# mcogoni/supersdr

Measured on AMD Instinct MI355X. Metric: real-time IQ channels sustained (WF+demod), higher is better.
Workload: dtype f32

## Files before the change

supersdr_amd/csrc/ssdr_wf.hip:

```cpp
#include "ssdr_math.h"
#include "ssdr_kernels.h"
#include "ssdr_audio_dev.h"
#include "ssdr_wf_dev.h"

namespace {

constexpr int WAVES = SSDR_WF_BLOCK / 64;
constexpr int LDS_TOTAL = LDS_XCH + WAVES * 2 * XCH_FLOATS * 4;
static_assert(LDS_TOTAL <= 163840, "LDS budget");
constexpr int LDS_SCAN = LDS_TOTAL;
constexpr int LDS_SCAN_BYTES = 6 * 64 * 4;
constexpr int LDS_TOTAL_FUSED = LDS_SCAN + LDS_SCAN_BYTES;
static_assert(LDS_SCAN % 4 == 0 && 2 * LDS_TOTAL_FUSED <= 163840, "two workgroups per CU");

template <bool AVG, bool HOP>
__global__ __launch_bounds__(SSDR_WF_BLOCK, SSDR_WF_WAVES_PER_EU) void ssdr_wf_kernel(SsdrWfArgs a)
{
    __shared__ __attribute__((aligned(16))) unsigned char smem[LDS_TOTAL];
    load_tables(smem, a.win, a.tw_stage, a.lut);

    const int lane = threadIdx.x & 63, wave = __builtin_amdgcn_readfirstlane(threadIdx.x >> 6);
    const int h = lane >> 5, l = lane & 31;
    float *xch_wave = reinterpret_cast<float *>(smem + LDS_XCH) + wave * 2 * XCH_FLOATS;
    const unsigned char *lut = smem + LDS_LUT0;
    const uint32_t n_pairs = (a.n_ch + 1) >> 1;
    const uint32_t run = HOP ? a.grp_run : 1u;
    const uint32_t n_runs = (a.n_groups + run - 1) / run;
    const uint32_t n_items = n_pairs * n_runs;
    const uint32_t wave_stride = gridDim.x * WAVES;

    for (uint32_t item = blockIdx.x * WAVES + wave; item < n_items; item += wave_stride) {
      uint32_t pair, g_begin, g_end;
      if (HOP) {
          pair = item / n_runs;
          g_begin = (item - pair * n_runs) * run;
          g_end = min(g_begin + run, a.n_groups);
      } else {
          g_begin = item / n_pairs;
          pair = item - g_begin * n_pairs;
          g_end = g_begin + 1;
      }
      const uint32_t n_trips = HOP ? g_end - g_begin : 1u;
      for (uint32_t trip = 0; trip < n_trips; trip++) {
        const uint32_t grp = g_begin + trip;
        uint32_t pair_now = __builtin_amdgcn_readfirstlane(pair);
        asm volatile("" : "+s"(pair_now));
        const WfItem it = wf_item(a, pair_now, grp, h);
        const float calq = a.consts[it.ch].wf_cal_lin * SSDR_LUT_SCALE;
        uint32_t acc[AVG ? 16 : 1];
#pragma unroll
        for (int j = 0; j < (AVG ? 16 : 1); j++) acc[j] = 0;
        constexpr uint32_t LINE_STEP = HOP ? SSDR_NFFT / 2 : SSDR_NFFT;
        const uint32_t *src = a.iq + (uint64_t)it.ch * a.ch_stride + (uint64_t)it.l0 * LINE_STEP + l;

        for (uint32_t line = it.l0; line < it.l1; line++, src += LINE_STEP) {
            f32x2 z[32];
            uint32_t raw[32];
            if (HOP) load_line_halves(line ? src - SSDR_NFFT / 2 : a.tail + (uint64_t)it.ch * (SSDR_NFFT / 2) + l, src, raw);
            else load_line(src, raw);
            if (SSDR_PRIO_WF) prio_compute_phase();
            window_line(raw, smem, l, z);
            SCHED_FENCE();
            fft_line<AVG>(z, smem, xch_wave, h, l);
            if (SSDR_PRIO_WF) prio_latency_phase();

            if (AVG) {
                quantise32(z, calq, lut, [&](int j, uint32_t q01) { acc[j] += q01; });
            } else {
                uint32_t q[16];
                quantise32(z, calq, lut, [&](int j, uint32_t q01) { q[j] = q01; });
                int16_t *x16 = reinterpret_cast<int16_t *>(xch_wave + opaque(h) * XCH_FLOATS) + opaque(l);
#pragma unroll
                for (int j = 0; j < 16; j++) {
                    x16[32 * (j + 16)] = (int16_t)(q[j] & 0xFFFFu);
                    x16[32 * j] = (int16_t)(q[j] >> 16);
                }
            }
        }

        float *xch = xch_wave + opaque(h) * XCH_FLOATS;
        if (AVG) {
            int16_t *x16 = reinterpret_cast<int16_t *>(xch) + opaque(l);
#pragma unroll
            for (int j = 0; j < 16; j++) {
                x16[32 * (j + 16)] = (int16_t)(acc[j] & 0xFFFFu);
                x16[32 * j] = (int16_t)(acc[j] >> 16);
            }
        }
        wave_lds_sync();
        const u32x4 *x128 = reinterpret_cast<const u32x4 *>(xch);
        int16_t *dst = it.complete ? a.out + ((uint64_t)it.grp * a.n_ch + it.ch) * SSDR_NFFT
                                   : a.acc_out + (uint64_t)it.ch * SSDR_NFFT;
        const int16_t *cin = a.acc_in + (uint64_t)it.ch * SSDR_NFFT;
#pragma unroll
        for (int q = 0; q < 4; q++) {
            u32x4 v = x128[q * 32 + l];
// ... 2 lines not shown
            if (it.ch_ok) SSDR_NT_STORE(v, reinterpret_cast<u32x4 *>(dst) + q * 32 + l);
        }
        wave_lds_sync();
      }
    }
}

template <typename T>
SSDR_DEV u32x4 *lane_at(T *base, uint32_t lane_bytes)
{
    return reinterpret_cast<u32x4 *>(reinterpret_cast<char *>(base) + lane_bytes);
}
template <typename T>
SSDR_DEV const u32x4 *lane_at(const T *base, uint32_t lane_bytes)
{
    return reinterpret_cast<const u32x4 *>(reinterpret_cast<const char *>(base) + lane_bytes);
}

template <bool HOP, bool AVG = false, bool HANG = true>
__global__ __launch_bounds__(SSDR_WF_BLOCK, SSDR_WF_WAVES_PER_EU) void ssdr_fused_am_kernel(SsdrFusedArgs fa)
{
    __shared__ __attribute__((aligned(16))) unsigned char smem[LDS_TOTAL_FUSED];
    const SsdrWfArgs &a = fa.wf;
    const SsdrAudioArgs &u = fa.au;
    if (threadIdx.x < 64) {
        DcScan t;
        scan_affine_consts(t);
        float *s_scan = reinterpret_cast<float *>(smem + LDS_SCAN) + threadIdx.x;
#pragma unroll
        for (int k = 1; k < 6; k++) s_scan[64 * (k - 1)] = t.a[k];
        s_scan[64 * 5] = t.ae;
    }
    load_tables(smem, a.win, a.tw_stage, a.lut);

    const int lane = threadIdx.x & 63, wave = __builtin_amdgcn_readfirstlane(threadIdx.x >> 6);
    const int h = lane >> 5, l = lane & 31;
    float *xch_wave = reinterpret_cast<float *>(smem + LDS_XCH) + wave * 2 * XCH_FLOATS;
    uint32_t *qbuf = reinterpret_cast<uint32_t *>(xch_wave);
    const unsigned char *lut = smem + LDS_LUT0;
    const uint32_t n_pairs = (a.n_ch + 1) >> 1;
    const uint32_t wave_stride = gridDim.x * WAVES;
    const uint32_t n_frames = u.n_frames;

    for (uint32_t pair = blockIdx.x * WAVES + wave; pair < n_pairs; pair += wave_stride) {
        const uint32_t ch_raw = 2 * pair + h;
        const bool ch_ok = ch_raw < a.n_ch;
        const uint32_t ch = ch_ok ? ch_raw : a.n_ch - 1;
        const float cal_wf = a.consts[ch].wf_cal_lin * SSDR_LUT_SCALE;
        const uint32_t n_sub = (2 * pair + 1 < a.n_ch) ? 2u : 1u;

        float rssi_sum[2] = {0.0f, 0.0f};
        uint32_t flag_keep[2] = {0u, 0u};
        auto pad = [&](int c, int i) -> float & { return xch_wave[c * XCH_FLOATS + 33 * (i + 17) + 32]; };
        constexpr int PAD_TAIL = HANG ? 10 : 2;
        constexpr bool PARKED = !HOP;
        constexpr int PARK = PARKED ? 4 : 0;
        if (lane < 2) {
            const uint32_t cc = min(2 * pair + (uint32_t)lane, a.n_ch - 1);
            const ssdr_chan_state st = u.state[cc];
            pad(lane, 0) = st.dc;
            pad(lane, 1) = st.agc_d;
            if (HANG) {
#pragma unroll
                for (int i = 0; i < 8; i++) pad(lane, 2 + i) = st.agc_m[i];
            }
            const uint4 t = *reinterpret_cast<const uint4 *>(u.hist + (size_t)cc * SSDR_HIST + SSDR_HIST - 4);
            if constexpr (PARKED) {
                pad(lane, PAD_TAIL) = __uint_as_float(t.x); pad(lane, PAD_TAIL + 1) = __uint_as_float(t.y);
                pad(lane, PAD_TAIL + 2) = __uint_as_float(t.z); pad(lane, PAD_TAIL + 3) = __uint_as_float(t.w);
            } else {
                pad(lane, PAD_TAIL) = __uint_as_float(iq_power(t.x)); pad(lane, PAD_TAIL + 1) = __uint_as_float(iq_power(t.y));
                pad(lane, PAD_TAIL + 2) = __uint_as_float(iq_power(t.z)); pad(lane, PAD_TAIL + 3) = __uint_as_float(iq_power(t.w));
            }
        }
        wave_lds_sync();

        const uint32_t *src = a.iq + (uint64_t)ch * a.ch_stride + l;
        uint32_t last_raw31 = 0;
        uint32_t acc[AVG ? 16 : 1];
#pragma unroll
        for (int j = 0; j < (AVG ? 16 : 1); j++) acc[j] = 0;
        constexpr uint32_t LINE_STEP = HOP ? SSDR_NFFT / 2 : SSDR_NFFT;
        constexpr int FRAMES_PER_LINE = HOP ? 1 : 2;
        for (uint32_t line = 0; line < a.n_lines; line++, src += LINE_STEP) {
            float dc[2], agc_d[2];
            AgcHang<HANG> hang[2];
            uint32_t tail_q[2][4];
#pragma unroll
            for (int c = 0; c < 2; c++) {
                dc[c] = pad(c, 0); agc_d[c] = pad(c, 1);
                if constexpr (HANG) {
#pragma unroll
                    for (int i = 0; i < 8; i++) hang[c].m[i] = pad(c, 2 + i);
                }
                if constexpr (!PARKED) {
#pragma unroll
                    for (int i = 0; i < 4; i++) tail_q[c][i] = __float_as_uint(pad(c, PAD_TAIL + i));
                }
            }
            if constexpr (PARKED) {
                u32x4 b[2];
#pragma unroll
                for (int c = 0; c < 2; c++)
#pragma unroll
                    for (int i = 0; i < 4; i++) b[c][i] = __float_as_uint(pad(c, PAD_TAIL + i));
                wave_lds_sync();
                if (lane == 0) {
#pragma unroll
                    for (int c = 0; c < 2; c++) *reinterpret_cast<u32x4 *>(qbuf + c * XCH_FLOATS) = b[c];
                }
            }
            wave_lds_sync();
            const uint32_t lw = opaque(lane);
            uint32_t *q_park = qbuf + PARK + 4 * lw;
            const uint32_t *q_lane = q_park - PARK + 4 * lw, *q_last = qbuf + (lw & 3u);
            const uint32_t lane16 = lw << 4;
            {
                u32x4 t[2][4];
#pragma unroll
                for (int c = 0; c < 2; c++) {
                    uint32_t pair_now = __builtin_amdgcn_readfirstlane(pair);
                    asm volatile("" : "+s"(pair_now));
                    const uint32_t cc = min(2 * pair_now + (uint32_t)c, a.n_ch - 1);
                    const uint32_t *row = a.iq + (uint64_t)cc * a.ch_stride + (uint64_t)line * LINE_STEP;
                    if (HOP) {
                        const uint32_t *older = line ? row - SSDR_NFFT / 2 : a.tail + (uint64_t)cc * (SSDR_NFFT / 2);
#pragma unroll
                        for (int i = 0; i < 2; i++) t[c][i] = SSDR_NT_LOAD(lane_at(older, lane16) + 64 * i);
#pragma unroll
                        for (int i = 0; i < 2; i++) t[c][2 + i] = lane_at(row, lane16)[64 * i];
                    } else {
#pragma unroll
                        for (int i = 0; i < 4; i++) t[c][i] = SSDR_NT_LOAD(lane_at(row, lane16) + 64 * i);
                    }
                }
                SCHED_FENCE();
#pragma unroll
                for (int c = 0; c < 2; c++)
#pragma unroll
                    for (int i = 0; i < 4; i++) reinterpret_cast<u32x4 *>(q_park + c * XCH_FLOATS)[64 * i] = t[c][i];
                SCHED_FENCE();
            }
            wave_lds_sync();
            DcScan dcs;
            {
                constexpr float DC_APOW[8] = SSDR_DC_APOW_INIT;
                uint32_t scan_base = LDS_SCAN;
                asm volatile("" : "+s"(scan_base));
                const float *s_scan = reinterpret_cast<const float *>(smem + scan_base) + lw;
                dcs.a[0] = DC_APOW[7];
                asm volatile("" : "+v"(dcs.a[0]));
#pragma unroll
                for (int k = 1; k < 6; k++) dcs.a[k] = s_scan[64 * (k - 1)];
                dcs.ae = s_scan[64 * 5];
            }
            prio_latency_phase();
#pragma unroll
            for (int c = 0; c < 2; c++) {
                if ((uint32_t)c >= n_sub) continue;
                uint32_t pair_now = __builtin_amdgcn_readfirstlane(pair);
                asm volatile("" : "+s"(pair_now));
                const uint32_t cc = 2 * pair_now + c;
                const ssdr_chan_consts &kc = u.consts[cc];
                const AgcK agc_c = {kc.agc_c0, kc.agc_c1, kc.agc_knee, kc.agc_delta8, kc.hang_frames};
                const float cal_c = kc.smeter_cal_db;
#pragma unroll
                for (int f = 0; f < FRAMES_PER_LINE; f++) {
                    const uint32_t frame = HOP ? line : 2 * line + f;
                    const int FBASE = c * XCH_FLOATS + SSDR_FRAME * (HOP ? 1 : f);
                    const u32x4 *qp = reinterpret_cast<const u32x4 *>(q_lane + FBASE);
                    const u32x4 q0 = qp[0], q1 = qp[1];
                    const uint32_t rw[8] = {q0.x, q0.y, q0.z, q0.w, q1.x, q1.y, q1.z, q1.w};
                    uint32_t d[8];
                    float p[8], aud[8];
                    float pmx;
                    bool trig;
                    uint32_t clip;
                    if constexpr (PARKED) {
                        const uint32_t last = q_last[FBASE + SSDR_FRAME];
#pragma unroll
                        for (int j = 0; j < 8; j++) d[j] = iq_power(rw[j]);
#pragma unroll
                        for (int j = 0; j < 8; j++) p[j] = (float)d[j];
                        pmx = block_peak(p);
                        trig = wave_any((pmx >= 1073676160.0f) | (iq_power(last) >= 0x3FFF0001u));
                        clip = trig ? (wave_count(raw_clipped_delayed(rw, last, lane)) + 63u) >> 6 : 0u;
                    } else {
                        uint32_t qv[8];
#pragma unroll
                        for (int j = 0; j < 8; j++) qv[j] = iq_power(rw[j]);
#pragma unroll
                        for (int j = 0; j < 4; j++) { d[j] = from_prev_lane_u(tail_q[c][j], qv[4 + j]); d[4 + j] = qv[j]; }
#pragma unroll
                        for (int j = 0; j < 4; j++) tail_q[c][j] = lane63_u(qv[4 + j]);
#pragma unroll
                        for (int j = 0; j < 8; j++) p[j] = (float)d[j];
                        pmx = block_peak(p);
                        trig = wave_any(pmx >= 1073676160.0f) || tail_q[c][0] >= 0x3FFF0001u || tail_q[c][1] >= 0x3FFF0001u ||
                               tail_q[c][2] >= 0x3FFF0001u || tail_q[c][3] >= 0x3FFF0001u;
                        clip = trig ? (wave_count(raw_clipped(rw)) + 63u) >> 6 : 0u;
                    }
                    demod_am_tab(p, dc[c], aud, dcs);
                    agc_pack_store_fused<HANG>(aud, lane, agc_c, agc_d[c], hang[c], u.pcm + ((uint64_t)cc * n_frames + frame) * SSDR_FRAME, lane16, pmx);
                    rssi_flag_step_uniform(p, clip, frame, n_frames, lane, cal_c, rssi_sum[c], flag_keep[c],
                                           u.rssi + (uint64_t)cc * n_frames, u.flags + (uint64_t)cc * n_frames);
                }
            }
            wave_lds_sync();
            prio_compute_phase();
            uint32_t raw[32];
            {
                const uint32_t *q = qbuf + opaque(h) * XCH_FLOATS + opaque(l);
#pragma unroll
                for (int r = 0; r < 32; r++) raw[r] = q[PARK + 32 * r];
            }
            wave_lds_sync();
            if (lane < 2) {
#pragma unroll
                for (int c = 0; c < 2; c++) {
                    if (lane != c) continue;
                    pad(c, 0) = dc[c]; pad(c, 1) = agc_d[c];
                    if constexpr (HANG) {
#pragma unroll
                        for (int i = 0; i < 8; i++) pad(c, 2 + i) = hang[c].m[i];
                    }
                    if constexpr (PARKED) {
                        const u32x4 e = *reinterpret_cast<const u32x4 *>(qbuf + c * XCH_FLOATS + PARK + SSDR_NFFT - 4);
#pragma unroll
                        for (int i = 0; i < 4; i++) pad(c, PAD_TAIL + i) = __uint_as_float(e[i]);
                    } else {
#pragma unroll
                        for (int i = 0; i < 4; i++) pad(c, PAD_TAIL + i) = __uint_as_float(tail_q[c][i]);
                    }
                }
            }
            wave_lds_sync();
            SCHED_FENCE();
            if (line + 1 == a.n_lines && ch_ok) {
#pragma unroll
                for (int r = 28; r < 32; r++) u.hist[(size_t)ch * SSDR_HIST + 32 * (r - 28) + l] = raw[r];
            }
            last_raw31 = raw[31];
            uint32_t qn[16];
            f32x2 z[32];
            window_line(raw, smem, l, z);
            SCHED_FENCE();
            fft_line<true>(z, smem, xch_wave, h, l);
            prio_latency_phase();
            if (AVG) quantise32(z, cal_wf, lut, [&](int j, uint32_t q01) { acc[j] += q01; });
            else quantise32(z, cal_wf, lut, [&](int j, uint32_t q01) { qn[j] = q01; });
            const uint32_t pos = a.phase + line;
            const bool group_done = !AVG || (pos + 1) % a.n_avg == 0;
            const bool last_line = line + 1 == a.n_lines;
            if (group_done || last_line) {
                float *xch = xch_wave + opaque(h) * XCH_FLOATS;
                int16_t *x16 = reinterpret_cast<int16_t *>(xch) + opaque(l);
#pragma unroll
                for (int j = 0; j < 16; j++) {
                    const uint32_t v = AVG ? acc[j] : qn[j];
                    x16[32 * (j + 16)] = (int16_t)(v & 0xFFFFu);
                    x16[32 * j] = (int16_t)(v >> 16);
                }
                wave_lds_sync();
                const u32x4 *x128 = reinterpret_cast<const u32x4 *>(xch);
                const uint32_t grp = AVG ? pos / a.n_avg : line;
                int16_t *dst = group_done ? a.out + ((uint64_t)grp * a.n_ch + ch) * SSDR_NFFT : a.acc_out + (uint64_t)ch * SSDR_NFFT;
                const bool carry_in = AVG && grp == 0 && a.phase != 0;
                const int16_t *cin = a.acc_in + (uint64_t)ch * SSDR_NFFT;
#pragma unroll
                for (int q = 0; q < 4; q++) {
                    u32x4 v = x128[q * 32 + l];
                    if (carry_in) v += reinterpret_cast<const u32x4 *>(cin)[q * 32 + l];
                    if (ch_ok) SSDR_NT_STORE(v, reinterpret_cast<u32x4 *>(dst) + q * 32 + l);
                }
                wave_lds_sync();
                if (AVG) {
#pragma unroll
                    for (int j = 0; j < 16; j++) acc[j] = 0;
                }
            }
        }

        if (a.n_lines) {
            uint32_t parg = 0;
#pragma unroll
            for (int c = 0; c < 2; c++) {
                if ((uint32_t)c >= n_sub) continue;
                const uint32_t cc = 2 * pair + c;
                const uint32_t dphi1 = u.consts[cc].dphi1;
                const uint32_t phi_last = u.state[cc].phi1 + (uint32_t)(SSDR_FRAME * (n_frames - 1)) * dphi1;
                parg = lane == 3 * c ? phi_last : lane == 3 * c + 1 ? (uint32_t)(8 * 63) * dphi1 : lane == 3 * c + 2 ? dphi1 : parg;
            }
            float pcos, psin;
            ssdr_phasor32(parg, pcos, psin);
#pragma unroll
            for (int c = 0; c < 2; c++) {
                if ((uint32_t)c >= n_sub) continue;
                const uint32_t cc = 2 * pair + c;
                const ssdr_chan_consts &kc = u.consts[cc];
                ssdr_chan_state st = u.state[cc];
                const float fc = lane_f(pcos, 3 * c), fs = lane_f(psin, 3 * c), qc = lane_f(pcos, 3 * c + 1), qs = lane_f(psin, 3 * c + 1);
                const float cs = lane_f(pcos, 3 * c + 2), ss = lane_f(psin, 3 * c + 2);
                float bc, bs;
                phasor_mul(fc, fs, qc, qs, bc, bs);
#pragma unroll
                for (int j = 0; j < 3; j++) { const float cn = fmaf(bc, cs, -(bs * ss)), sn = fmaf(bs, cs, bc * ss); bc = cn; bs = sn; }
                const float xr = (float)(int16_t)(last_raw31 & 0xFFFFu), xi = (float)((int32_t)last_raw31 >> 16);
                const float zr = fmaf(xr, bc, xi * bs) + 0.0f, zi = fmaf(xi, bc, -(xr * bs)) + 0.0f;
                st.prev_re = lane_f(zr, 32 * c + 27);
                st.prev_im = lane_f(zi, 32 * c + 27);
                st.phi1 += (uint32_t)(SSDR_FRAME * n_frames) * kc.dphi1;
                st.phi2 += (uint32_t)(SSDR_FRAME * n_frames) * kc.dphi2;
                st.dc = pad(c, 0); st.agc_d = pad(c, 1);
                if (HANG) {
#pragma unroll
                    for (int i = 0; i < 8; i++) st.agc_m[i] = pad(c, 2 + i);
                }
                if (lane == 0) u.state[cc] = st;
            }
        }
    }
}

__global__ __launch_bounds__(256) void ssdr_quant_selftest_kernel(const float *thr_g, const uint32_t *lut_g,
                                                                    unsigned long long *mismatch)
{
    __shared__ __attribute__((aligned(16))) unsigned char smem[LDS_LUT_END + 16 + 1024];
    float *s_thr = reinterpret_cast<float *>(smem + ((LDS_LUT_END + 15) & ~15));
    uint32_t *s_lut = reinterpret_cast<uint32_t *>(smem + LDS_LUT0);
    for (int i = threadIdx.x; i < 256; i += blockDim.x) s_thr[i] = thr_g[i];
    for (int i = threadIdx.x; i < SSDR_LUT_N; i += blockDim.x) s_lut[i] = lut_g[i];
    __syncthreads();
    unsigned long long bad = 0;
    const unsigned char *lut = smem + LDS_LUT0;
    const uint64_t stride = (uint64_t)gridDim.x * blockDim.x;
    for (uint64_t u = (uint64_t)blockIdx.x * blockDim.x + threadIdx.x; u < 0x7F800000ull; u += stride) {
        const float p = __uint_as_float((uint32_t)u);
        int lo = 0, hi = 255;
        while (lo < hi) {
            const int mid = (lo + hi + 1) >> 1;
            if (s_thr[mid] <= p) lo = mid; else hi = mid - 1;
        }
        float pc;
        asm("v_mul_f32_e64 %0, %1, %2 clamp" : "=v"(pc) : "v"(p), "v"(SSDR_LUT_SCALE));
        bad += (quantise(pc, lut) != (uint32_t)lo);
    }
    if (bad) atomicAdd(mismatch, bad);
}

}

// ... 71 lines not shown
```

supersdr_amd/csrc/ssdr_wf_dev.h:

```cpp
#pragma once
#include "ssdr_math.h"
#include "ssdr_kernels.h"

namespace {

constexpr int XPAD = 33;
constexpr int XCH_FLOATS = 32 * XPAD;
typedef uint32_t u32x4 __attribute__((ext_vector_type(4)));
typedef float f32x2 __attribute__((ext_vector_type(2)));

constexpr int LDS_WIN = 0;
constexpr int LDS_LUT0 = 2064;
constexpr int LDS_LUT_END = LDS_LUT0 + SSDR_LUT_N * 4;
constexpr int LDS_TW = (LDS_LUT_END + 15) & ~15;
constexpr int LDS_XCH = LDS_TW + SSDR_TW_STAGE_N * 8;
static_assert(LDS_XCH % 16 == 0 && LDS_TW % 8 == 0, "alignment");

#define SCHED_FENCE() __builtin_amdgcn_sched_barrier(0)

#ifndef SSDR_PRIO
#define SSDR_PRIO 1
#endif
#ifndef SSDR_PRIO_WF
#define SSDR_PRIO_WF 1
// ... 31 lines not shown
SSDR_DEV void stage_const(f32x2 (&z)[32])
{
    constexpr float W32R[16] = SSDR_W32R_INIT;
    constexpr float W32I[16] = SSDR_W32I_INIT;
    constexpr int half = 1 << (S - 1);
#pragma unroll
    for (int k = 0; k < half; k++) {
        const int mi = k * (32 >> S);
#pragma unroll
        for (int blk = 0; blk < 32; blk += 2 * half) {
            const int i = blk + k, j = i + half;
            if (mi == 0) bfly_1(z[i], z[j]);
            else if (mi == 8) bfly_mj(z[i], z[j]);
            else bfly(z[i], z[j], W32R[mi], W32I[mi]);
        }
    }
}

template <int T, int JL0, int NJL>
SSDR_DEV void stage_lane(f32x2 (&z)[32], const f32x2 (&w)[NJL])
{
    constexpr int half = 1 << T;
#pragma unroll
    for (int q = 0; q < NJL; q++) {
        const int jl = JL0 + q;
#pragma unroll
        for (int blk = 0; blk < 32; blk += 2 * half) {
            const int i = blk + jl, j = i + half;
            bfly(z[i], z[j], w[q].x, w[q].y);
        }
    }
}

template <int T, int JL0, int NJL>
SSDR_DEV void load_tw(f32x2 (&w)[NJL], const f32x2 *tw_lane)
{
    constexpr int off = 32 * ((1 << T) - 1);
#pragma unroll
    for (int q = 0; q < NJL; q++) w[q] = tw_lane[off + (JL0 + q) * 32];
}

SSDR_DEV int opaque(int v)
{
    asm volatile("" : "+v"(v));
    return v;
}

SSDR_DEV float *opaque_lds(float *p)
{
    typedef __attribute__((address_space(3))) float lds_float;
    uint32_t a = (uint32_t)(uintptr_t)(lds_float *)p;
    asm volatile("" : "+v"(a));
    return (float *)(lds_float *)(uintptr_t)a;
}

SSDR_DEV void wave_lds_sync()
{
    __builtin_amdgcn_fence(__ATOMIC_RELEASE, "wavefront");
    __builtin_amdgcn_wave_barrier();
    __builtin_amdgcn_fence(__ATOMIC_ACQUIRE, "wavefront");
}

SSDR_DEV float quant_scaled_power(f32x2 z, float calq)
{
    float p = fmaf(z.x, z.x, z.y * z.y), pc;
    asm("v_mul_f32_e64 %0, %1, %2 clamp" : "=v"(pc) : "v"(p), "v"(calq));
    return pc;
}
SSDR_DEV uint32_t quant_addr(float pc) { return (__float_as_uint(pc) >> (SSDR_LUT_SHIFT - 2)) & ~3u; }
SSDR_DEV uint32_t quant_word(float pc, uint32_t w) { return __float_as_uint(pc) + w; }
SSDR_DEV uint32_t quant_pair(uint32_t w0, uint32_t w1) { return __builtin_amdgcn_perm(w1, w0, 0x0C070C03u); }
SSDR_DEV uint32_t quantise(float p_scaled_clamped, const unsigned char *lut)
// ... 66 lines not shown
SSDR_DEV void window_line(const uint32_t (&raw)[32], const unsigned char *smem, int l, f32x2 (&z)[32])
{
    const int ll = opaque(l);
    const float *win_up = reinterpret_cast<const float *>(smem + LDS_WIN) + ll;
    const float *win_dn = reinterpret_cast<const float *>(smem + LDS_WIN) - ll;
    f32x2 wu[8], wd[8];
#pragma unroll
    for (int k = 0; k < 8; k++) {
        wu[k] = f32x2{win_up[32 * (2 * k)], win_up[32 * (2 * k + 1)]};
        wd[k] = f32x2{win_dn[32 * (16 - (2 * k + 1))], win_dn[32 * (16 - 2 * k)]};
    }
    SCHED_FENCE();
#pragma unroll
    for (int k = 0; k < 8; k++) {
#pragma unroll
        for (int hh = 0; hh < 2; hh++) {
            const int r = 2 * k + hh;
            const f32x2 xa = {(float)(int16_t)(raw[r] & 0xFFFFu), (float)((int32_t)raw[r] >> 16)};
            const f32x2 xb = {(float)(int16_t)(raw[r + 16] & 0xFFFFu), (float)((int32_t)raw[r + 16] >> 16)};
            if (hh == 0) {
                const f32x2 t = pk_mul_half<0>(xa, wu[k]);
                z[brev5(r)] = pk_fma_half<1, false>(xb, wd[k], t);
                z[brev5(r) + 1] = pk_fma_half<1, true>(xb, wd[k], t);
            } else {
                const f32x2 t = pk_mul_half<1>(xa, wu[k]);
                z[brev5(r)] = pk_fma_half<0, false>(xb, wd[k], t);
                z[brev5(r) + 1] = pk_fma_half<0, true>(xb, wd[k], t);
            }
        }
        if (k & 1) SCHED_FENCE();
    }
}

template <bool TIGHT>
SSDR_DEV void fft_line(f32x2 (&z)[32], const unsigned char *smem, float *xch_wave, int h, int l)
{
    stage_const<2>(z);
    stage_const<3>(z);
    stage_const<4>(z);
    stage_const<5>(z);
    SCHED_FENCE();

    const int lx = opaque(l);
    float *xch = xch_wave + opaque(h) * XCH_FLOATS;
    const int g = __builtin_bitreverse32((uint32_t)lx) >> 27;
    float *row = opaque_lds(xch + g * XPAD);
#pragma unroll
    for (int r = 0; r < 32; r++) row[r] = z[r].x;
    wave_lds_sync();
#pragma unroll
    for (int j = 0; j < 32; j++) z[j].x = xch[j * XPAD + lx];
    wave_lds_sync();
#pragma unroll
    for (int r = 0; r < 32; r++) row[r] = z[r].y;
    wave_lds_sync();
#pragma unroll
    for (int j = 0; j < 32; j++) z[j].y = xch[j * XPAD + lx];
    wave_lds_sync();

    const f32x2 *s_tw_lane = reinterpret_cast<const f32x2 *>(smem + LDS_TW) + opaque(l);
    f32x2 w0[1], w1[2], w2[4];
    load_tw<0, 0, 1>(w0, s_tw_lane);
    load_tw<1, 0, 2>(w1, s_tw_lane);
    load_tw<2, 0, 4>(w2, s_tw_lane);
    SCHED_FENCE();
    stage_lane<0, 0, 1>(z, w0);
    stage_lane<1, 0, 2>(z, w1);
    if (!TIGHT) {
        f32x2 w3[8];
        load_tw<3, 0, 8>(w3, s_tw_lane);
        SCHED_FENCE();
        stage_lane<2, 0, 4>(z, w2);
        SCHED_FENCE();
        f32x2 w4a[8];
        load_tw<4, 0, 8>(w4a, s_tw_lane);
        SCHED_FENCE();
        stage_lane<3, 0, 8>(z, w3);
        SCHED_FENCE();
        f32x2 w4b[8];
        load_tw<4, 8, 8>(w4b, s_tw_lane);
        SCHED_FENCE();
        stage_lane<4, 0, 8>(z, w4a);
        SCHED_FENCE();
        stage_lane<4, 8, 8>(z, w4b);
        SCHED_FENCE();
    } else {
        f32x2 wa[4], wb[4];
        load_tw<3, 0, 4>(wa, s_tw_lane);
        SCHED_FENCE();
        stage_lane<2, 0, 4>(z, w2);
        SCHED_FENCE();
        load_tw<3, 4, 4>(wb, s_tw_lane);
        SCHED_FENCE();
        stage_lane<3, 0, 4>(z, wa);
        SCHED_FENCE();
        load_tw<4, 0, 4>(wa, s_tw_lane);
        SCHED_FENCE();
        stage_lane<3, 4, 4>(z, wb);
        SCHED_FENCE();
        load_tw<4, 4, 4>(wb, s_tw_lane);
        SCHED_FENCE();
        stage_lane<4, 0, 4>(z, wa);
        SCHED_FENCE();
        load_tw<4, 8, 4>(wa, s_tw_lane);
        SCHED_FENCE();
        stage_lane<4, 4, 4>(z, wb);
        SCHED_FENCE();
        load_tw<4, 12, 4>(wb, s_tw_lane);
        SCHED_FENCE();
        stage_lane<4, 8, 4>(z, wa);
        SCHED_FENCE();
        stage_lane<4, 12, 4>(z, wb);
        SCHED_FENCE();
    }
}

struct WfItem {
    uint32_t ch, l0, l1, grp;
    bool ch_ok, carry_in, complete;
};

SSDR_DEV WfItem wf_item(const SsdrWfArgs &a, uint32_t pair, uint32_t grp, int h)
{
    WfItem it;
    it.grp = grp;
    const uint32_t ch_raw = 2 * pair + h;
    it.ch_ok = ch_raw < a.n_ch;
    it.ch = it.ch_ok ? ch_raw : a.n_ch - 1;
    const int64_t g0 = (int64_t)it.grp * a.n_avg - a.phase;
    it.l0 = g0 < 0 ? 0u : (uint32_t)g0;
    it.l1 = min((uint32_t)(g0 + a.n_avg), a.n_lines);
    it.carry_in = (it.grp == 0) && (a.phase != 0);
    it.complete = (g0 + (int64_t)a.n_avg) <= (int64_t)a.n_lines;
    return it;
}

SSDR_DEV void load_tables(unsigned char *smem, const float *win, const float2 *tw, const uint32_t *lut)
{
    float *s_win = reinterpret_cast<float *>(smem + LDS_WIN);
    f32x2 *s_tw = reinterpret_cast<f32x2 *>(smem + LDS_TW);
    uint32_t *s_lut = reinterpret_cast<uint32_t *>(smem + LDS_LUT0);
    for (int i = threadIdx.x; i < 513; i += blockDim.x) s_win[i] = win[i];
    for (int i = threadIdx.x; i < SSDR_TW_STAGE_N; i += blockDim.x) s_tw[i] = f32x2{tw[i].x, tw[i].y};
    for (int i = threadIdx.x; i < SSDR_LUT_N; i += blockDim.x) s_lut[i] = lut[i];
// ... 5 lines not shown
```

Before: 46.25 million.

## Prefetch first line IQ with state loads and stage per-pair phase words in LDS

The fused AM kernel now issues the first line's IQ loads together with the per-channel state, history and consts loads in the prologue, so their latencies overlap. Phase words needed at the epilogue are precomputed into a new per-wave LDS area, and the state record is written back with vector stores from two lanes instead of repeated global re-reads. It also adds an early exit when n_lines is zero and moves the latency-priority hint inside the per-channel loop. The cost is extra LDS and register pressure from keeping the prefetched tile live across the loop, which depends on the state struct layout matching the u32x4 indexing.

```diff
diff --git a/supersdr_amd/csrc/ssdr_wf.hip b/supersdr_amd/csrc/ssdr_wf.hip
--- a/supersdr_amd/csrc/ssdr_wf.hip
+++ b/supersdr_amd/csrc/ssdr_wf.hip
@@ -10,8 +10,11 @@
 static_assert(LDS_TOTAL <= 163840, "LDS budget");
 constexpr int LDS_SCAN = LDS_TOTAL;
 constexpr int LDS_SCAN_BYTES = 6 * 64 * 4;
-constexpr int LDS_TOTAL_FUSED = LDS_SCAN + LDS_SCAN_BYTES;
-static_assert(LDS_SCAN % 4 == 0 && 2 * LDS_TOTAL_FUSED <= 163840, "two workgroups per CU");
+constexpr int LDS_PAIR = LDS_SCAN + LDS_SCAN_BYTES;
+enum { PAIR_PHI_LAST, PAIR_DPHI_504, PAIR_DPHI, PAIR_PHI1, PAIR_PHI2, PAIR_WORDS };
+constexpr int LDS_PAIR_BYTES = WAVES * 2 * PAIR_WORDS * 4;
+constexpr int LDS_TOTAL_FUSED = LDS_PAIR + LDS_PAIR_BYTES;
+static_assert(LDS_SCAN % 4 == 0 && LDS_PAIR % 16 == 0 && 2 * LDS_TOTAL_FUSED <= 163840, "two workgroups per CU");
 
 template <bool AVG, bool HOP>
 __global__ __launch_bounds__(SSDR_WF_BLOCK, SSDR_WF_WAVES_PER_EU) void ssdr_wf_kernel(SsdrWfArgs a)
@@ -130,6 +133,7 @@
         s_scan[64 * 5] = t.ae;
     }
     load_tables(smem, a.win, a.tw_stage, a.lut);
+    if (a.n_lines == 0) return;
 
     const int lane = threadIdx.x & 63, wave = __builtin_amdgcn_readfirstlane(threadIdx.x >> 6);
     const int h = lane >> 5, l = lane & 31;
@@ -153,22 +157,54 @@
         constexpr int PAD_TAIL = HANG ? 10 : 2;
         constexpr bool PARKED = !HOP;
         constexpr int PARK = PARKED ? 4 : 0;
-        if (lane < 2) {
-            const uint32_t cc = min(2 * pair + (uint32_t)lane, a.n_ch - 1);
-            const ssdr_chan_state st = u.state[cc];
-            pad(lane, 0) = st.dc;
-            pad(lane, 1) = st.agc_d;
-            if (HANG) {
-#pragma unroll
-                for (int i = 0; i < 8; i++) pad(lane, 2 + i) = st.agc_m[i];
-            }
-            const uint4 t = *reinterpret_cast<const uint4 *>(u.hist + (size_t)cc * SSDR_HIST + SSDR_HIST - 4);
-            if constexpr (PARKED) {
-                pad(lane, PAD_TAIL) = __uint_as_float(t.x); pad(lane, PAD_TAIL + 1) = __uint_as_float(t.y);
-                pad(lane, PAD_TAIL + 2) = __uint_as_float(t.z); pad(lane, PAD_TAIL + 3) = __uint_as_float(t.w);
-            } else {
-                pad(lane, PAD_TAIL) = __uint_as_float(iq_power(t.x)); pad(lane, PAD_TAIL + 1) = __uint_as_float(iq_power(t.y));
-                pad(lane, PAD_TAIL + 2) = __uint_as_float(iq_power(t.z)); pad(lane, PAD_TAIL + 3) = __uint_as_float(iq_power(t.w));
+        constexpr uint32_t LINE_STEP = HOP ? SSDR_NFFT / 2 : SSDR_NFFT;
+        constexpr int FRAMES_PER_LINE = HOP ? 1 : 2;
+        auto issue_line = [&](uint32_t line, uint32_t lane16, u32x4 (&t)[2][4]) {
+#pragma unroll
+            for (int c = 0; c < 2; c++) {
+                uint32_t pair_now = __builtin_amdgcn_readfirstlane(pair);
+                asm volatile("" : "+s"(pair_now));
+                const uint32_t cc = min(2 * pair_now + (uint32_t)c, a.n_ch - 1);
+                const uint32_t *row = a.iq + (uint64_t)cc * a.ch_stride + (uint64_t)line * LINE_STEP;
+                if (HOP) {
+                    const uint32_t *older = line ? row - SSDR_NFFT / 2 : a.tail + (uint64_t)cc * (SSDR_NFFT / 2);
+#pragma unroll
+                    for (int i = 0; i < 2; i++) t[c][i] = SSDR_NT_LOAD(lane_at(older, lane16) + 64 * i);
+#pragma unroll
+                    for (int i = 0; i < 2; i++) t[c][2 + i] = lane_at(row, lane16)[64 * i];
+                } else {
+#pragma unroll
+                    for (int i = 0; i < 4; i++) t[c][i] = SSDR_NT_LOAD(lane_at(row, lane16) + 64 * i);
+                }
+            }
+        };
+        u32x4 t[2][4];
+        {
+            const int ln = opaque(lane);
+            const uint32_t cc = min(2 * pair + ((uint32_t)ln & 1u), a.n_ch - 1);
+            const u32x4 *rec = reinterpret_cast<const u32x4 *>(u.state + cc);
+            const u32x4 s0 = rec[0];
+            u32x4 m[2];
+            if constexpr (HANG) { m[0] = rec[1]; m[1] = rec[2]; }
+            const u32x4 tl = *reinterpret_cast<const u32x4 *>(u.hist + (size_t)cc * SSDR_HIST + SSDR_HIST - 4);
+            const uint32_t dphi1 = u.consts[cc].dphi1, dphi2 = u.consts[cc].dphi2;
+            issue_line(0, (uint32_t)ln << 4, t);
+            wave_lds_sync();
+            if (ln < 2) {
+                pad(ln, 0) = __uint_as_float(s0[2]);
+                pad(ln, 1) = __uint_as_float(s0[3]);
+                if constexpr (HANG) {
+#pragma unroll
+                    for (int i = 0; i < 8; i++) pad(ln, 2 + i) = __uint_as_float(m[i >> 2][i & 3]);
+                }
+#pragma unroll
+                for (int i = 0; i < 4; i++) pad(ln, PAD_TAIL + i) = __uint_as_float(PARKED ? tl[i] : iq_power(tl[i]));
+                uint32_t *cell = reinterpret_cast<uint32_t *>(smem + LDS_PAIR) + (2 * wave + ln) * PAIR_WORDS;
+                cell[PAIR_PHI_LAST] = s0[0] + (uint32_t)(SSDR_FRAME * (n_frames - 1)) * dphi1;
+                cell[PAIR_DPHI_504] = (uint32_t)(8 * 63) * dphi1;
+                cell[PAIR_DPHI] = dphi1;
+                cell[PAIR_PHI1] = s0[0] + (uint32_t)(SSDR_FRAME * n_frames) * dphi1;
+                cell[PAIR_PHI2] = s0[1] + (uint32_t)(SSDR_FRAME * n_frames) * dphi2;
             }
         }
         wave_lds_sync();
@@ -178,8 +214,6 @@
         uint32_t acc[AVG ? 16 : 1];
 #pragma unroll
         for (int j = 0; j < (AVG ? 16 : 1); j++) acc[j] = 0;
-        constexpr uint32_t LINE_STEP = HOP ? SSDR_NFFT / 2 : SSDR_NFFT;
-        constexpr int FRAMES_PER_LINE = HOP ? 1 : 2;
         for (uint32_t line = 0; line < a.n_lines; line++, src += LINE_STEP) {
             float dc[2], agc_d[2];
             AgcHang<HANG> hang[2];
@@ -214,24 +248,7 @@
             const uint32_t *q_lane = q_park - PARK + 4 * lw, *q_last = qbuf + (lw & 3u);
             const uint32_t lane16 = lw << 4;
             {
-                u32x4 t[2][4];
-#pragma unroll
-                for (int c = 0; c < 2; c++) {
-                    uint32_t pair_now = __builtin_amdgcn_readfirstlane(pair);
-                    asm volatile("" : "+s"(pair_now));
-                    const uint32_t cc = min(2 * pair_now + (uint32_t)c, a.n_ch - 1);
-                    const uint32_t *row = a.iq + (uint64_t)cc * a.ch_stride + (uint64_t)line * LINE_STEP;
-                    if (HOP) {
-                        const uint32_t *older = line ? row - SSDR_NFFT / 2 : a.tail + (uint64_t)cc * (SSDR_NFFT / 2);
-#pragma unroll
-                        for (int i = 0; i < 2; i++) t[c][i] = SSDR_NT_LOAD(lane_at(older, lane16) + 64 * i);
-#pragma unroll
-                        for (int i = 0; i < 2; i++) t[c][2 + i] = lane_at(row, lane16)[64 * i];
-                    } else {
-#pragma unroll
-                        for (int i = 0; i < 4; i++) t[c][i] = SSDR_NT_LOAD(lane_at(row, lane16) + 64 * i);
-                    }
-                }
+                if (line) issue_line(line, lane16, t);
                 SCHED_FENCE();
 #pragma unroll
                 for (int c = 0; c < 2; c++)
@@ -252,7 +269,6 @@
                 for (int k = 1; k < 6; k++) dcs.a[k] = s_scan[64 * (k - 1)];
                 dcs.ae = s_scan[64 * 5];
             }
-            prio_latency_phase();
 #pragma unroll
             for (int c = 0; c < 2; c++) {
                 if ((uint32_t)c >= n_sub) continue;
@@ -262,6 +278,7 @@
                 const ssdr_chan_consts &kc = u.consts[cc];
                 const AgcK agc_c = {kc.agc_c0, kc.agc_c1, kc.agc_knee, kc.agc_delta8, kc.hang_frames};
                 const float cal_c = kc.smeter_cal_db;
+                prio_latency_phase();
 #pragma unroll
                 for (int f = 0; f < FRAMES_PER_LINE; f++) {
                     const uint32_t frame = HOP ? line : 2 * line + f;
@@ -377,26 +394,22 @@
                     for (int j = 0; j < 16; j++) acc[j] = 0;
                 }
             }
-        }
-
-        if (a.n_lines) {
-            uint32_t parg = 0;
+#pragma unroll
+            for (int c = 0; c < 2; c++)
+#pragma unroll
+                for (int i = 0; i < 4; i++) asm volatile("" : "=v"(t[c][i]));
+        }
+
+        {
+            const uint32_t *cells = reinterpret_cast<const uint32_t *>(smem + LDS_PAIR) + 2 * wave * PAIR_WORDS;
+            const int ln = opaque(lane);
+            const uint32_t parg = cells[ln < 3 ? ln : ln < 6 ? ln + (PAIR_WORDS - 3) : 0];
+            float pcos, psin;
+            ssdr_phasor32(parg, pcos, psin);
+            float prev_re = 0.0f, prev_im = 0.0f;
 #pragma unroll
             for (int c = 0; c < 2; c++) {
                 if ((uint32_t)c >= n_sub) continue;
-                const uint32_t cc = 2 * pair + c;
-                const uint32_t dphi1 = u.consts[cc].dphi1;
-                const uint32_t phi_last = u.state[cc].phi1 + (uint32_t)(SSDR_FRAME * (n_frames - 1)) * dphi1;
-                parg = lane == 3 * c ? phi_last : lane == 3 * c + 1 ? (uint32_t)(8 * 63) * dphi1 : lane == 3 * c + 2 ? dphi1 : parg;
-            }
-            float pcos, psin;
-            ssdr_phasor32(parg, pcos, psin);
-#pragma unroll
-            for (int c = 0; c < 2; c++) {
-                if ((uint32_t)c >= n_sub) continue;
-                const uint32_t cc = 2 * pair + c;
-                const ssdr_chan_consts &kc = u.consts[cc];
-                ssdr_chan_state st = u.state[cc];
                 const float fc = lane_f(pcos, 3 * c), fs = lane_f(psin, 3 * c), qc = lane_f(pcos, 3 * c + 1), qs = lane_f(psin, 3 * c + 1);
                 const float cs = lane_f(pcos, 3 * c + 2), ss = lane_f(psin, 3 * c + 2);
                 float bc, bs;
@@ -405,16 +418,21 @@
                 for (int j = 0; j < 3; j++) { const float cn = fmaf(bc, cs, -(bs * ss)), sn = fmaf(bs, cs, bc * ss); bc = cn; bs = sn; }
                 const float xr = (float)(int16_t)(last_raw31 & 0xFFFFu), xi = (float)((int32_t)last_raw31 >> 16);
                 const float zr = fmaf(xr, bc, xi * bs) + 0.0f, zi = fmaf(xi, bc, -(xr * bs)) + 0.0f;
-                st.prev_re = lane_f(zr, 32 * c + 27);
-                st.prev_im = lane_f(zi, 32 * c + 27);
-                st.phi1 += (uint32_t)(SSDR_FRAME * n_frames) * kc.dphi1;
-                st.phi2 += (uint32_t)(SSDR_FRAME * n_frames) * kc.dphi2;
-                st.dc = pad(c, 0); st.agc_d = pad(c, 1);
-                if (HANG) {
-#pragma unroll
-                    for (int i = 0; i < 8; i++) st.agc_m[i] = pad(c, 2 + i);
-                }
-                if (lane == 0) u.state[cc] = st;
+                const float re_c = lane_f(zr, 32 * c + 27), im_c = lane_f(zi, 32 * c + 27);
+                prev_re = ln == c ? re_c : prev_re;
+                prev_im = ln == c ? im_c : prev_im;
+            }
+            if ((uint32_t)ln < n_sub) {
+                u32x4 *rec = reinterpret_cast<u32x4 *>(u.state + (2 * pair + (uint32_t)ln));
+                const uint32_t *cell = cells + ln * PAIR_WORDS;
+                rec[0] = u32x4{cell[PAIR_PHI1], cell[PAIR_PHI2], __float_as_uint(pad(ln, 0)), __float_as_uint(pad(ln, 1))};
+                if constexpr (HANG) {
+                    u32x4 m[2];
+#pragma unroll
+                    for (int i = 0; i < 8; i++) m[i >> 2][i & 3] = __float_as_uint(pad(ln, 2 + i));
+                    rec[1] = m[0]; rec[2] = m[1];
+                }
+                *reinterpret_cast<float2 *>(rec + 3) = float2{prev_re, prev_im};
             }
         }
     }
```

Measured after the change: 46.59 million, median of 6. About the same (+0.7%).

## Use ds_write_addtid row stores and inline-asm twiddle reads in FFT transpose

Applied to the files above, without the earlier changes.

Replaces the per-lane bit-reversed row stores in the FFT's LDS transpose with ds_write_addtid_b32 instructions addressed through M0 and immediate offsets. Each wave's scratch becomes a 65-float-pitch row layout read back by bit-reversed column. Twiddle loads become hand-written ds_read_b64 sequences with immediate offsets and explicit lgkmcnt waits. The fused AM kernel's per-wave buffer map, channel pad slots and queue offsets are re-laid out to fit the new scheme. The aim is to cut VALU address arithmetic and LDS instruction overhead in the transpose. The risk is that the explicit waitcnts and M0 use constrain the compiler's scheduling.

```diff
diff --git a/supersdr_amd/csrc/ssdr_wf.hip b/supersdr_amd/csrc/ssdr_wf.hip
--- a/supersdr_amd/csrc/ssdr_wf.hip
+++ b/supersdr_amd/csrc/ssdr_wf.hip
@@ -5,9 +5,17 @@
 
 namespace {
 
+#ifndef SSDR_WF_LDS_FORMS
+#define SSDR_WF_LDS_FORMS 1
+#endif
 constexpr int WAVES = SSDR_WF_BLOCK / 64;
 constexpr int LDS_TOTAL = LDS_XCH + WAVES * 2 * XCH_FLOATS * 4;
 static_assert(LDS_TOTAL <= 163840, "LDS budget");
+constexpr int CH_FLOATS = 4 + SSDR_NFFT;
+constexpr int FUSED_REST = XROWS_FLOATS;
+constexpr int FUSED_WAVE_FLOATS = 2 * XCH_FLOATS;
+static_assert(2 * CH_FLOATS <= XROWS_FLOATS && FUSED_REST + 32 <= FUSED_WAVE_FLOATS && (CH_FLOATS * 4) % 16 == 0, "the wave buffer's map");
+static_assert((WAVES - 1) * FUSED_WAVE_FLOATS * 4 < 65536, "the wave's distance from LDS_XCH fits M0's 16 address bits");
 constexpr int LDS_SCAN = LDS_TOTAL;
 constexpr int LDS_SCAN_BYTES = 6 * 64 * 4;
 constexpr int LDS_TOTAL_FUSED = LDS_SCAN + LDS_SCAN_BYTES;
@@ -61,7 +69,8 @@
             if (SSDR_PRIO_WF) prio_compute_phase();
             window_line(raw, smem, l, z);
             SCHED_FENCE();
-            fft_line<AVG>(z, smem, xch_wave, h, l);
+            constexpr bool FORMS = SSDR_WF_LDS_FORMS && !(AVG && HOP);
+            fft_line<AVG, FORMS, FORMS>(z, smem, xch_wave, h, l);
             if (SSDR_PRIO_WF) prio_latency_phase();
 
             if (AVG) {
@@ -133,7 +142,7 @@
 
     const int lane = threadIdx.x & 63, wave = __builtin_amdgcn_readfirstlane(threadIdx.x >> 6);
     const int h = lane >> 5, l = lane & 31;
-    float *xch_wave = reinterpret_cast<float *>(smem + LDS_XCH) + wave * 2 * XCH_FLOATS;
+    float *xch_wave = reinterpret_cast<float *>(smem + LDS_XCH) + wave * FUSED_WAVE_FLOATS;
     uint32_t *qbuf = reinterpret_cast<uint32_t *>(xch_wave);
     const unsigned char *lut = smem + LDS_LUT0;
     const uint32_t n_pairs = (a.n_ch + 1) >> 1;
@@ -149,8 +158,10 @@
 
         float rssi_sum[2] = {0.0f, 0.0f};
         uint32_t flag_keep[2] = {0u, 0u};
-        auto pad = [&](int c, int i) -> float & { return xch_wave[c * XCH_FLOATS + 33 * (i + 17) + 32]; };
         constexpr int PAD_TAIL = HANG ? 10 : 2;
+        auto pad = [&](int c, int i) -> float & {
+            return xch_wave[FUSED_REST + (i >= PAD_TAIL ? 4 * c + (i - PAD_TAIL) : i < 2 ? 8 + 2 * c + i : 12 + 8 * c + (i - 2))];
+        };
         constexpr bool PARKED = !HOP;
         constexpr int PARK = PARKED ? 4 : 0;
         if (lane < 2) {
@@ -205,7 +216,7 @@
                 wave_lds_sync();
                 if (lane == 0) {
 #pragma unroll
-                    for (int c = 0; c < 2; c++) *reinterpret_cast<u32x4 *>(qbuf + c * XCH_FLOATS) = b[c];
+                    for (int c = 0; c < 2; c++) *reinterpret_cast<u32x4 *>(qbuf + c * CH_FLOATS) = b[c];
                 }
             }
             wave_lds_sync();
@@ -236,7 +247,7 @@
 #pragma unroll
                 for (int c = 0; c < 2; c++)
 #pragma unroll
-                    for (int i = 0; i < 4; i++) reinterpret_cast<u32x4 *>(q_park + c * XCH_FLOATS)[64 * i] = t[c][i];
+                    for (int i = 0; i < 4; i++) reinterpret_cast<u32x4 *>(q_park + c * CH_FLOATS)[64 * i] = t[c][i];
                 SCHED_FENCE();
             }
             wave_lds_sync();
@@ -265,7 +276,7 @@
 #pragma unroll
                 for (int f = 0; f < FRAMES_PER_LINE; f++) {
                     const uint32_t frame = HOP ? line : 2 * line + f;
-                    const int FBASE = c * XCH_FLOATS + SSDR_FRAME * (HOP ? 1 : f);
+                    const int FBASE = c * CH_FLOATS + SSDR_FRAME * (HOP ? 1 : f);
                     const u32x4 *qp = reinterpret_cast<const u32x4 *>(q_lane + FBASE);
                     const u32x4 q0 = qp[0], q1 = qp[1];
                     const uint32_t rw[8] = {q0.x, q0.y, q0.z, q0.w, q1.x, q1.y, q1.z, q1.w};
@@ -308,7 +319,7 @@
             prio_compute_phase();
             uint32_t raw[32];
             {
-                const uint32_t *q = qbuf + opaque(h) * XCH_FLOATS + opaque(l);
+                const uint32_t *q = qbuf + opaque(h) * CH_FLOATS + opaque(l);
 #pragma unroll
                 for (int r = 0; r < 32; r++) raw[r] = q[PARK + 32 * r];
             }
@@ -323,7 +334,7 @@
                         for (int i = 0; i < 8; i++) pad(c, 2 + i) = hang[c].m[i];
                     }
                     if constexpr (PARKED) {
-                        const u32x4 e = *reinterpret_cast<const u32x4 *>(qbuf + c * XCH_FLOATS + PARK + SSDR_NFFT - 4);
+                        const u32x4 e = *reinterpret_cast<const u32x4 *>(qbuf + c * CH_FLOATS + PARK + SSDR_NFFT - 4);
 #pragma unroll
                         for (int i = 0; i < 4; i++) pad(c, PAD_TAIL + i) = __uint_as_float(e[i]);
                     } else {
@@ -343,7 +354,7 @@
             f32x2 z[32];
             window_line(raw, smem, l, z);
             SCHED_FENCE();
-            fft_line<true>(z, smem, xch_wave, h, l);
+            fft_line<true, true, true>(z, smem, xch_wave, h, l);
             prio_latency_phase();
             if (AVG) quantise32(z, cal_wf, lut, [&](int j, uint32_t q01) { acc[j] += q01; });
             else quantise32(z, cal_wf, lut, [&](int j, uint32_t q01) { qn[j] = q01; });
@@ -351,7 +362,7 @@
             const bool group_done = !AVG || (pos + 1) % a.n_avg == 0;
             const bool last_line = line + 1 == a.n_lines;
             if (group_done || last_line) {
-                float *xch = xch_wave + opaque(h) * XCH_FLOATS;
+                float *xch = xch_wave + opaque(h) * CH_FLOATS;
                 int16_t *x16 = reinterpret_cast<int16_t *>(xch) + opaque(l);
 #pragma unroll
                 for (int j = 0; j < 16; j++) {
diff --git a/supersdr_amd/csrc/ssdr_wf_dev.h b/supersdr_amd/csrc/ssdr_wf_dev.h
--- a/supersdr_amd/csrc/ssdr_wf_dev.h
+++ b/supersdr_amd/csrc/ssdr_wf_dev.h
@@ -87,12 +87,49 @@
     }
 }
 
-template <int T, int JL0, int NJL>
-SSDR_DEV void load_tw(f32x2 (&w)[NJL], const f32x2 *tw_lane)
-{
-    constexpr int off = 32 * ((1 << T) - 1);
-#pragma unroll
-    for (int q = 0; q < NJL; q++) w[q] = tw_lane[off + (JL0 + q) * 32];
+template <int B>
+SSDR_DEV void tw_read1(f32x2 &a, uint32_t tw_addr)
+{
+    asm volatile("ds_read_b64 %0, %1 offset:%2" : "=&v"(a) : "v"(tw_addr), "n"(B));
+}
+template <int B>
+SSDR_DEV void tw_read2(f32x2 &a, f32x2 &b, uint32_t tw_addr)
+{
+    asm volatile("ds_read_b64 %0, %2 offset:%3\n\tds_read_b64 %1, %2 offset:%4" : "=&v"(a), "=&v"(b) : "v"(tw_addr), "n"(B), "n"(B + 256));
+}
+template <int B>
+SSDR_DEV void tw_read4(f32x2 &a, f32x2 &b, f32x2 &c, f32x2 &d, uint32_t tw_addr)
+{
+    asm volatile("ds_read_b64 %0, %4 offset:%5\n\tds_read_b64 %1, %4 offset:%6\n\tds_read_b64 %2, %4 offset:%7\n\tds_read_b64 %3, %4 offset:%8"
+                 : "=&v"(a), "=&v"(b), "=&v"(c), "=&v"(d) : "v"(tw_addr), "n"(B), "n"(B + 256), "n"(B + 512), "n"(B + 768));
+}
+template <int T, int JL0, int NJL, bool TW1>
+SSDR_DEV void load_tw(f32x2 (&w)[NJL], uint32_t tw_addr )
+{
+    constexpr int B = 256 * ((1 << T) - 1 + JL0);
+    static_assert(NJL == 1 || NJL == 2 || NJL == 4 || NJL == 8, "group size");
+    static_assert(B + 256 * NJL <= SSDR_TW_STAGE_N * 8, "inside the table");
+    if constexpr (!TW1) {
+        typedef __attribute__((address_space(3))) const f32x2 lds_f32x2;
+        const f32x2 *t = (const f32x2 *)(lds_f32x2 *)(uintptr_t)tw_addr;
+#pragma unroll
+        for (int q = 0; q < NJL; q++) w[q] = t[B / 8 + 32 * q];
+        return;
+    }
+    if constexpr (NJL == 1) tw_read1<B>(w[0], tw_addr);
+    if constexpr (NJL == 2) tw_read2<B>(w[0], w[1], tw_addr);
+    if constexpr (NJL >= 4) tw_read4<B>(w[0], w[1], w[2], w[3], tw_addr);
+    if constexpr (NJL == 8) tw_read4<B + 1024>(w[4], w[5], w[6], w[7], tw_addr);
+}
+template <bool TW1, bool WAIT = true, int NJL>
+SSDR_DEV void tw_ready(f32x2 (&w)[NJL])
+{
+    if constexpr (!TW1) return;
+    if constexpr (WAIT) asm volatile("s_waitcnt lgkmcnt(0)" : : : "memory");
+    if constexpr (NJL == 1) asm volatile("" : "+v"(w[0]));
+    if constexpr (NJL == 2) asm volatile("" : "+v"(w[0]), "+v"(w[1]));
+    if constexpr (NJL >= 4) asm volatile("" : "+v"(w[0]), "+v"(w[1]), "+v"(w[2]), "+v"(w[3]));
+    if constexpr (NJL == 8) asm volatile("" : "+v"(w[4]), "+v"(w[5]), "+v"(w[6]), "+v"(w[7]));
 }
 
 SSDR_DEV int opaque(int v)
@@ -225,7 +262,35 @@
     }
 }
 
-template <bool TIGHT>
+constexpr int XROW = 65;
+constexpr int XROWS_FLOATS = 32 * XROW;
+#pragma clang diagnostic ignored "-Winline-asm"
+template <int R0, int C>
+SSDR_DEV void xrows_store8(const f32x2 (&z)[32], uint32_t m0_wave)
+{
+    static_assert(LDS_XCH + 4 * XROW * 31 < 65536, "offset field");
+    auto v = [&](int r) { return C ? z[r].y : z[r].x; };
+    asm volatile("s_mov_b32 m0, %8\n\ts_nop 0\n\t"
+                 "ds_write_addtid_b32 %0 offset:%9\n\tds_write_addtid_b32 %1 offset:%10\n\tds_write_addtid_b32 %2 offset:%11\n\t"
+                 "ds_write_addtid_b32 %3 offset:%12\n\tds_write_addtid_b32 %4 offset:%13\n\tds_write_addtid_b32 %5 offset:%14\n\t"
+                 "ds_write_addtid_b32 %6 offset:%15\n\tds_write_addtid_b32 %7 offset:%16"
+                 : : "v"(v(R0)), "v"(v(R0 + 1)), "v"(v(R0 + 2)), "v"(v(R0 + 3)), "v"(v(R0 + 4)), "v"(v(R0 + 5)), "v"(v(R0 + 6)), "v"(v(R0 + 7)),
+                     "s"(m0_wave),
+                     "n"(LDS_XCH + 4 * XROW * R0), "n"(LDS_XCH + 4 * XROW * (R0 + 1)), "n"(LDS_XCH + 4 * XROW * (R0 + 2)),
+                     "n"(LDS_XCH + 4 * XROW * (R0 + 3)), "n"(LDS_XCH + 4 * XROW * (R0 + 4)), "n"(LDS_XCH + 4 * XROW * (R0 + 5)),
+                     "n"(LDS_XCH + 4 * XROW * (R0 + 6)), "n"(LDS_XCH + 4 * XROW * (R0 + 7))
+                 : "memory", "m0");
+}
+template <int C>
+SSDR_DEV void xrows_store(const f32x2 (&z)[32], uint32_t m0_wave)
+{
+    xrows_store8<0, C>(z, m0_wave);
+    xrows_store8<8, C>(z, m0_wave);
+    xrows_store8<16, C>(z, m0_wave);
+    xrows_store8<24, C>(z, m0_wave);
+}
+
+template <bool TIGHT, bool XROWS = false, bool TW1 = false>
 SSDR_DEV void fft_line(f32x2 (&z)[32], const unsigned char *smem, float *xch_wave, int h, int l)
 {
     stage_const<2>(z);
@@ -234,75 +299,106 @@
     stage_const<5>(z);
     SCHED_FENCE();
 
+    typedef __attribute__((address_space(3))) const unsigned char lds_byte;
+    typedef __attribute__((address_space(3))) float lds_float;
     const int lx = opaque(l);
-    float *xch = xch_wave + opaque(h) * XCH_FLOATS;
-    const int g = __builtin_bitreverse32((uint32_t)lx) >> 27;
-    float *row = opaque_lds(xch + g * XPAD);
-#pragma unroll
-    for (int r = 0; r < 32; r++) row[r] = z[r].x;
-    wave_lds_sync();
-#pragma unroll
-    for (int j = 0; j < 32; j++) z[j].x = xch[j * XPAD + lx];
-    wave_lds_sync();
-#pragma unroll
-    for (int r = 0; r < 32; r++) row[r] = z[r].y;
-    wave_lds_sync();
-#pragma unroll
-    for (int j = 0; j < 32; j++) z[j].y = xch[j * XPAD + lx];
-    wave_lds_sync();
-
-    const f32x2 *s_tw_lane = reinterpret_cast<const f32x2 *>(smem + LDS_TW) + opaque(l);
+    if constexpr (XROWS) {
+        uint32_t xch_addr = __builtin_amdgcn_readfirstlane((uint32_t)(uintptr_t)(lds_float *)xch_wave);
+        asm volatile("" : "+s"(xch_addr));
+        const uint32_t m0_wave = xch_addr - (uint32_t)(uintptr_t)(lds_byte *)(smem + LDS_XCH);
+        const float *col = opaque_lds(xch_wave + (lx * XROW + opaque(h) * 32));
+        xrows_store<0>(z, m0_wave);
+        wave_lds_sync();
+#pragma unroll
+        for (int j = 0; j < 32; j++) z[j].x = col[brev5(j)];
+        wave_lds_sync();
+        xrows_store<1>(z, m0_wave);
+        wave_lds_sync();
+#pragma unroll
+        for (int j = 0; j < 32; j++) z[j].y = col[brev5(j)];
+        wave_lds_sync();
+    } else {
+        float *xch = xch_wave + opaque(h) * XCH_FLOATS;
+        const int g = __builtin_bitreverse32((uint32_t)lx) >> 27;
+        float *row = opaque_lds(xch + g * XPAD);
+#pragma unroll
+        for (int r = 0; r < 32; r++) row[r] = z[r].x;
+        wave_lds_sync();
+#pragma unroll
+        for (int j = 0; j < 32; j++) z[j].x = xch[j * XPAD + lx];
+        wave_lds_sync();
+#pragma unroll
+        for (int r = 0; r < 32; r++) row[r] = z[r].y;
+        wave_lds_sync();
+#pragma unroll
+        for (int j = 0; j < 32; j++) z[j].y = xch[j * XPAD + lx];
+        wave_lds_sync();
+    }
+
+    const uint32_t tw_addr = (uint32_t)(uintptr_t)(lds_byte *)(smem + LDS_TW) + 8u * (uint32_t)opaque(l);
     f32x2 w0[1], w1[2], w2[4];
-    load_tw<0, 0, 1>(w0, s_tw_lane);
-    load_tw<1, 0, 2>(w1, s_tw_lane);
-    load_tw<2, 0, 4>(w2, s_tw_lane);
+    load_tw<0, 0, 1, TW1>(w0, tw_addr);
+    load_tw<1, 0, 2, TW1>(w1, tw_addr);
+    load_tw<2, 0, 4, TW1>(w2, tw_addr);
+    tw_ready<TW1>(w0);
+    tw_ready<TW1, false>(w1);
+    tw_ready<TW1, false>(w2);
     SCHED_FENCE();
     stage_lane<0, 0, 1>(z, w0);
     stage_lane<1, 0, 2>(z, w1);
     if (!TIGHT) {
         f32x2 w3[8];
-        load_tw<3, 0, 8>(w3, s_tw_lane);
+        load_tw<3, 0, 8, TW1>(w3, tw_addr);
         SCHED_FENCE();
         stage_lane<2, 0, 4>(z, w2);
         SCHED_FENCE();
         f32x2 w4a[8];
-        load_tw<4, 0, 8>(w4a, s_tw_lane);
+        tw_ready<TW1>(w3);
+        load_tw<4, 0, 8, TW1>(w4a, tw_addr);
         SCHED_FENCE();
         stage_lane<3, 0, 8>(z, w3);
         SCHED_FENCE();
         f32x2 w4b[8];
-        load_tw<4, 8, 8>(w4b, s_tw_lane);
+        tw_ready<TW1>(w4a);
+        load_tw<4, 8, 8, TW1>(w4b, tw_addr);
         SCHED_FENCE();
         stage_lane<4, 0, 8>(z, w4a);
         SCHED_FENCE();
+        tw_ready<TW1>(w4b);
         stage_lane<4, 8, 8>(z, w4b);
         SCHED_FENCE();
     } else {
         f32x2 wa[4], wb[4];
-        load_tw<3, 0, 4>(wa, s_tw_lane);
+        load_tw<3, 0, 4, TW1>(wa, tw_addr);
         SCHED_FENCE();
         stage_lane<2, 0, 4>(z, w2);
         SCHED_FENCE();
-        load_tw<3, 4, 4>(wb, s_tw_lane);
+        tw_ready<TW1>(wa);
+        load_tw<3, 4, 4, TW1>(wb, tw_addr);
         SCHED_FENCE();
         stage_lane<3, 0, 4>(z, wa);
         SCHED_FENCE();
-        load_tw<4, 0, 4>(wa, s_tw_lane);
+        tw_ready<TW1>(wb);
+        load_tw<4, 0, 4, TW1>(wa, tw_addr);
         SCHED_FENCE();
         stage_lane<3, 4, 4>(z, wb);
         SCHED_FENCE();
-        load_tw<4, 4, 4>(wb, s_tw_lane);
+        tw_ready<TW1>(wa);
+        load_tw<4, 4, 4, TW1>(wb, tw_addr);
         SCHED_FENCE();
         stage_lane<4, 0, 4>(z, wa);
         SCHED_FENCE();
-        load_tw<4, 8, 4>(wa, s_tw_lane);
+        tw_ready<TW1>(wb);
+        load_tw<4, 8, 4, TW1>(wa, tw_addr);
         SCHED_FENCE();
         stage_lane<4, 4, 4>(z, wb);
         SCHED_FENCE();
-        load_tw<4, 12, 4>(wb, s_tw_lane);
+        tw_ready<TW1>(wa);
+        load_tw<4, 12, 4, TW1>(wb, tw_addr);
         SCHED_FENCE();
         stage_lane<4, 8, 4>(z, wa);
         SCHED_FENCE();
+        tw_ready<TW1>(wb);
         stage_lane<4, 12, 4>(z, wb);
         SCHED_FENCE();
     }
```

After: 45.17 million before, 45.55 million after (median of 6 runs). No clear change (+0.8%).
